# barbararoessle/e2e_multi_view_matching

Hardware: NVIDIA H100
Metric: view-tuples/sec @1024 kpts 5-view (higher is better)
Workload: dtype f32 via split operands on the tensor cores (fp16x3 / tf32x3, fp32-faithful) / f64 pose kernels

## Files before the change

e2e_multi_view_matching_b200/csrc/gemm_tc.cu:

```cuda
#include <cstring>
#include <map>
#include <mutex>
#include <tuple>
#include <cuda_fp16.h>
#include "common.cuh"
#include "kernels.cuh"
#include "tc_common.cuh"

namespace {

constexpr int BM = 128;
constexpr int PRODUCER_WARP = 8;
constexpr int NTHREADS = 384;
constexpr int PRODUCER_REGS = 40, CONSUMER_REGS = 232;
enum { W_RAW = 0, W_TF32 = 1, W_F16 = 2 };

template <int BN, int NPASS, int WM>
struct Cfg {
  static constexpr int BK = WM == W_F16 ? 64 : 32;
  static constexpr int A_BYTES = BM * BK * 4;
  static constexpr int W_PLANE = BN * 128;
  static constexpr int PLANES = NPASS == 3 ? 2 : 1;
  static constexpr int STAGE_BYTES = A_BYTES + PLANES * W_PLANE;
  static constexpr int TMA_BYTES = A_BYTES + (WM == W_RAW ? 1 : PLANES) * W_PLANE;
  static constexpr int STAGES = (196608 / STAGE_BYTES) < 6 ? (196608 / STAGE_BYTES) : 6;
  static constexpr bool STAGED = BN == 128 && NPASS == 3 && WM != W_RAW;
  static constexpr int OUT_BYTES = STAGED ? 2 * 16384 : 0;
  static constexpr int SMEM_BYTES = STAGES * STAGE_BYTES + OUT_BYTES + 1024  + 256 ;
  static_assert(SMEM_BYTES <= 232448, "over the sm_90 dynamic shared memory opt-in limit");
};

struct GArgs {
  const float* bias;
  const float* R; int ldr;
  float* C; int ldc;
  int M, N, K, K1;
  float alpha;
  int relu;
  float* VT; int vt_col0; int n_pad;
  float* KLO; float* VTLO;
  __half* KH16; __half* KL16; __half* VH16; __half* VL16;
  int tiles_m, tiles_n;
  int ksplit;
  int stage;
};

struct StoreMaps {
  CUtensorMap c, r, p[4];
};

struct ScoreTab {
  int n_pairs, batch, n_views, n_pad;
  int a[MVM_MAX_PAIRS], b[MVM_MAX_PAIRS], m[MVM_MAX_PAIRS], n[MVM_MAX_PAIRS];
  float* scores[MVM_MAX_PAIRS];
};

__device__ __forceinline__ float tf32_hi(float x) {
  return __uint_as_float((__float_as_uint(x) + 0x1000u) & 0xffffe000u);
}
__device__ __forceinline__ void split_pack_h(float x0, float x1, uint32_t& hi, uint32_t& lo) {
  const __half2 h = __floats2half2_rn(x0, x1);
  const float2 hf = __half22float2(h);
  const __half2 l = __floats2half2_rn(x0 - hf.x, x1 - hf.y);
  hi = *reinterpret_cast<const uint32_t*>(&h);
  lo = *reinterpret_cast<const uint32_t*>(&l);
}
__device__ __forceinline__ void sts_f2(uint32_t a, float2 v) {
  asm volatile("st.shared.v2.f32 [%0], {%1, %2};" ::"r"(a), "f"(v.x), "f"(v.y) : "memory");
}
__device__ __forceinline__ void sts_u32(uint32_t a, uint32_t v) {
  asm volatile("st.shared.b32 [%0], %1;" ::"r"(a), "r"(v) : "memory");
}
__device__ __forceinline__ float2 lds_f2(uint32_t a) {
  float2 v;
  asm volatile("ld.shared.v2.f32 {%0, %1}, [%2];" : "=f"(v.x), "=f"(v.y) : "r"(a) : "memory");
  return v;
}
__device__ __forceinline__ void fence_afrag(uint32_t (&a)[4][4]) {
#pragma unroll
  for (int i = 0; i < 4; ++i)
#pragma unroll
    for (int e = 0; e < 4; ++e) asm volatile("" : "+r"(a[i][e])::"memory");
}

template <int BN, int NPASS, int WM, bool SCORE>
__global__ void __launch_bounds__(NTHREADS, 1)
gemm_wg_kernel(const __grid_constant__ CUtensorMap tmA, const __grid_constant__ CUtensorMap tmA2,
               const __grid_constant__ CUtensorMap tmWhi, const __grid_constant__ CUtensorMap tmWlo,
               const __grid_constant__ GArgs g, const __grid_constant__ ScoreTab st,
               const __grid_constant__ StoreMaps sm) {
  using C_ = Cfg<BN, NPASS, WM>;
  static_assert(NPASS == 3 || WM == W_RAW, "single pass reads the raw W");
  constexpr int BK = C_::BK, STAGES = C_::STAGES, A_BYTES = C_::A_BYTES, W_PLANE = C_::W_PLANE;
  constexpr int STAGE_BYTES = C_::STAGE_BYTES;
  constexpr int KSTEPS = 4;
  constexpr bool PIPE = BN == 128;
  constexpr bool STAGED = C_::STAGED && !SCORE;
  extern __shared__ uint8_t smem_raw[];
  uint8_t* smem = reinterpret_cast<uint8_t*>((reinterpret_cast<uintptr_t>(smem_raw) + 1023) & ~uintptr_t(1023));
  uint8_t* obuf = smem + STAGES * STAGE_BYTES;
  uint64_t* full = reinterpret_cast<uint64_t*>(obuf + C_::OUT_BYTES);
  uint64_t* empty = full + STAGES;
  uint64_t* ostaged = empty + STAGES;
  uint64_t* ofree = ostaged + 2;

  const int warp = threadIdx.x >> 5, lane = threadIdx.x & 31;
  const int nk = SCORE ? g.K / BK : g.K / BK / g.ksplit;
  const int per_prob = g.tiles_m * g.tiles_n;
  const int n_tiles = SCORE ? per_prob * st.n_pairs * st.batch : per_prob * g.ksplit;
  auto decode = [&](int tile, int& m0, int& n0, int& a_row, int& w_row, int& prob) {
    prob = tile / per_prob;
    const int r = tile % per_prob;
    m0 = (r / g.tiles_n) * BM; n0 = (r % g.tiles_n) * BN;
    if (!SCORE) {
      a_row = m0; w_row = n0;
    } else {
      const int p = prob / st.batch, bi = prob % st.batch;
      a_row = (bi * st.n_views + st.a[p]) * st.n_pad + m0;
      w_row = (bi * st.n_views + st.b[p]) * st.n_pad + n0;
    }
  };
  auto tile_kind = [&](int n0) {
    if (g.VT && n0 >= g.vt_col0) return -1;
    if (g.KH16 && n0 >= 256) return 1;
    if (g.KLO && n0 >= 256 && n0 < 512) return 2;
    return 0;
  };

  if (threadIdx.x == 0) {
    for (int s = 0; s < STAGES; ++s) {
      tc::mbar_init(full + s, 1);
      tc::mbar_init(empty + s, 256);
    }
    if (STAGED)
      for (int b = 0; b < 2; ++b) {
        tc::mbar_init(ostaged + b, 256);
        tc::mbar_init(ofree + b, 1);
      }
    tc::fence_barrier_init();
  }
  __syncthreads();

  if (warp >= PRODUCER_WARP) {
    asm volatile("setmaxnreg.dec.sync.aligned.u32 %0;" ::"n"(PRODUCER_REGS));
    if (STAGED && g.stage && warp == PRODUCER_WARP + 1 && lane == 0) {
      tc::prefetch_tmap(&sm.c);
      if (g.R) tc::prefetch_tmap(&sm.r);
      if (g.KH16)
        for (int i = 0; i < 4; ++i) tc::prefetch_tmap(&sm.p[i]);
      if (g.KLO) tc::prefetch_tmap(&sm.p[0]);
      auto hand_back = [&](uint32_t u, int tile, int q) {
        uint64_t* bar = ofree + (u & 1);
        if (!g.R) {
          tc::mbar_arrive(bar);
        } else if (tile < n_tiles) {
          int m0, n0, a_row, w_row, prob;
          decode(tile, m0, n0, a_row, w_row, prob);
          tc::mbar_arrive_expect_tx(bar, 16384);
          tc::tma_load_2d(obuf + (u & 1) * 16384, &sm.r, bar, n0 + 32 * q, m0);
        }
      };
      hand_back(0, blockIdx.x, 0);
      hand_back(1, blockIdx.x, 1);
      uint32_t u = 0;
      for (int tile = blockIdx.x; tile < n_tiles; tile += gridDim.x) {
        int m0, n0, a_row, w_row, prob;
        decode(tile, m0, n0, a_row, w_row, prob);
        const int kind = tile_kind(n0);
        if (kind < 0) continue;
        const int rounds = kind == 2 ? 8 : 4;
        for (int j = 0; j < rounds; ++j, ++u) {
          const uint8_t* buf = obuf + (u & 1) * 16384;
          tc::mbar_wait(ostaged + (u & 1), (u >> 1) & 1);
          if (kind == 0) {
            tc::tma_store_2d(&sm.c, buf, n0 + 32 * j, m0 + prob * g.tiles_m * BM);
          } else if (kind == 1) {
            const bool v = n0 >= 512;
            tc::tma_store_2d(&sm.p[(v ? 2 : 0) + (j & 1)], buf, n0 - (v ? 512 : 256) + 64 * (j >> 1), m0);
          } else {
            if (j & 1) tc::tma_store_2d(&sm.p[0], buf, n0 - 256 + 32 * (j >> 1), m0);
            else tc::tma_store_2d(&sm.c, buf, n0 + 32 * (j >> 1), m0);
          }
          tc::tma_store_commit();
          tc::tma_store_wait_read<0>();
          hand_back(u + 2, j < 2 ? tile : tile + gridDim.x, (j + 2) & 3);
        }
      }
      tc::tma_store_wait_all();
    }
    if (warp == PRODUCER_WARP && lane == 0) {
      tc::prefetch_tmap(&tmA); tc::prefetch_tmap(&tmA2); tc::prefetch_tmap(&tmWhi); tc::prefetch_tmap(&tmWlo);
      uint32_t it = 0;
      for (int tile = blockIdx.x; tile < n_tiles; tile += gridDim.x) {
        int m0, n0, a_row, w_row, prob;
        decode(tile, m0, n0, a_row, w_row, prob);
        for (int kt = 0; kt < nk; ++kt, ++it) {
          const int s = it % STAGES;
          tc::mbar_wait(empty + s, ((it / STAGES) & 1) ^ 1);
          tc::mbar_arrive_expect_tx(full + s, C_::TMA_BYTES);
          uint8_t* sp = smem + s * STAGE_BYTES;
          const int k = kt * BK + (SCORE ? 0 : prob * nk * BK);
          if (k < g.K1) tc::tma_load_2d(sp, &tmA, full + s, k, a_row);
          else tc::tma_load_2d(sp, &tmA2, full + s, k - g.K1, a_row);
          if (WM == W_F16) {
            if (k < g.K1) tc::tma_load_2d(sp + 16384, &tmA, full + s, k + 32, a_row);
            else tc::tma_load_2d(sp + 16384, &tmA2, full + s, k + 32 - g.K1, a_row);
          }
          tc::tma_load_2d(sp + A_BYTES, &tmWhi, full + s, k, w_row);
          if (WM != W_RAW) tc::tma_load_2d(sp + A_BYTES + W_PLANE, &tmWlo, full + s, k, w_row);
        }
      }
    }
    return;
  }

  asm volatile("setmaxnreg.inc.sync.aligned.u32 %0;" ::"n"(CONSUMER_REGS));
  const int wg = warp >> 2, wq = warp & 3;
  const int gr = lane >> 2, tq = lane & 3;
  const int row0 = wg * 64 + wq * 16 + gr;
  float acc[BN / 2];
  uint32_t ahi0[KSTEPS][4], alo0[KSTEPS][4], ahi1[KSTEPS][4], alo1[KSTEPS][4];

  auto prep = [&](uint32_t it, uint32_t (&ahi)[KSTEPS][4], uint32_t (&alo)[KSTEPS][4]) {
      const int s = it % STAGES;
      tc::mbar_wait(full + s, (it / STAGES) & 1);
      uint8_t* sp = smem + s * STAGE_BYTES;
      if (WM == W_RAW && NPASS == 3) {
        float4* w = reinterpret_cast<float4*>(sp + A_BYTES);
        float4* wl = reinterpret_cast<float4*>(sp + A_BYTES + W_PLANE);
#pragma unroll 4
        for (int i = threadIdx.x; i < BN * 32 / 4; i += 256) {
          const float4 x = w[i];
          float4 h;
          h.x = tc::tf32_rn(x.x); h.y = tc::tf32_rn(x.y); h.z = tc::tf32_rn(x.z); h.w = tc::tf32_rn(x.w);
          w[i] = h;
          wl[i] = make_float4(tc::tf32_rn(x.x - h.x), tc::tf32_rn(x.y - h.y), tc::tf32_rn(x.z - h.z), tc::tf32_rn(x.w - h.w));
        }
        tc::fence_proxy_async();
        asm volatile("bar.sync 1, 256;" ::: "memory");
      }
      const uint8_t* ar = sp + row0 * 128;
#pragma unroll
      for (int kk = 0; kk < KSTEPS; ++kk) {
        if (WM == W_F16) {
          const uint8_t* ab = ar + (kk >> 1) * 16384;
          const int ch = 4 * (kk & 1) + (tq >> 1), wo = (tq & 1) * 8;
          const float2 x0 = *reinterpret_cast<const float2*>(ab + ((ch ^ gr) << 4) + wo);
          const float2 x1 = *reinterpret_cast<const float2*>(ab + 1024 + ((ch ^ gr) << 4) + wo);
          const float2 x2 = *reinterpret_cast<const float2*>(ab + (((ch + 2) ^ gr) << 4) + wo);
          const float2 x3 = *reinterpret_cast<const float2*>(ab + 1024 + (((ch + 2) ^ gr) << 4) + wo);
          split_pack_h(x0.x, x0.y, ahi[kk][0], alo[kk][0]);
          split_pack_h(x1.x, x1.y, ahi[kk][1], alo[kk][1]);
          split_pack_h(x2.x, x2.y, ahi[kk][2], alo[kk][2]);
          split_pack_h(x3.x, x3.y, ahi[kk][3], alo[kk][3]);
        } else {
          float x[4];
          x[0] = *reinterpret_cast<const float*>(ar + (((2 * kk) ^ gr) << 4) + tq * 4);
          x[1] = *reinterpret_cast<const float*>(ar + 1024 + (((2 * kk) ^ gr) << 4) + tq * 4);
          x[2] = *reinterpret_cast<const float*>(ar + (((2 * kk + 1) ^ gr) << 4) + tq * 4);
          x[3] = *reinterpret_cast<const float*>(ar + 1024 + (((2 * kk + 1) ^ gr) << 4) + tq * 4);
#pragma unroll
          for (int e = 0; e < 4; ++e) {
            if (NPASS == 3) {
              const float h = tf32_hi(x[e]);
              ahi[kk][e] = __float_as_uint(h);
              alo[kk][e] = __float_as_uint(tf32_hi(x[e] - h));
            } else {
              ahi[kk][e] = __float_as_uint(x[e]);
            }
          }
        }
      }
  };
  auto issue = [&](uint32_t it, const uint32_t (&ahi)[KSTEPS][4], const uint32_t (&alo)[KSTEPS][4]) {
      const uint32_t whi = tc::smem_u32(smem + (it % STAGES) * STAGE_BYTES + A_BYTES);
      tc::wgmma_fence();
#pragma unroll
      for (int kk = 0; kk < KSTEPS; ++kk) {
#pragma unroll
        for (int nh = 0; nh < BN / 128; ++nh) {
          float* d = acc + nh * 64;
          const uint32_t wb = whi + nh * 16384 + kk * 32;
          if (WM == W_F16) {
            tc::wgmma_f16_rs<128, 0>(d, ahi[kk], tc::make_sw128_desc(wb));
            tc::wgmma_f16_rs<128, 0>(d, ahi[kk], tc::make_sw128_desc(wb + W_PLANE));
            tc::wgmma_f16_rs<128, 0>(d, alo[kk], tc::make_sw128_desc(wb));
          } else {
            tc::wgmma_tf32_rs<128>(d, ahi[kk], tc::make_sw128_desc(wb));
            if (NPASS == 3) {
              tc::wgmma_tf32_rs<128>(d, ahi[kk], tc::make_sw128_desc(wb + W_PLANE));
              tc::wgmma_tf32_rs<128>(d, alo[kk], tc::make_sw128_desc(wb));
            }
          }
        }
      }
      tc::wgmma_commit();
  };
  auto keep = [&](uint32_t (&ahi)[KSTEPS][4], uint32_t (&alo)[KSTEPS][4]) {
    fence_afrag(ahi);
    if (NPASS == 3) fence_afrag(alo);
  };

  auto stage_round = [&](uint32_t u, int n0, int i0, int ni, int mode, int plane) {
    const uint32_t buf = tc::smem_u32(obuf + (u & 1) * 16384);
    float2 bv[8];
#pragma unroll
    for (int c = 0; c < ni; ++c) {
      const int n = n0 + 8 * (i0 + c) + 2 * tq;
      bv[c] = g.bias ? make_float2(__ldg(g.bias + n), __ldg(g.bias + n + 1)) : make_float2(0.f, 0.f);
    }
    tc::mbar_wait(ofree + (u & 1), (u >> 1) & 1);
#pragma unroll
    for (int c = 0; c < ni; ++c) {
      const int i = i0 + c;
#pragma unroll
      for (int hh = 0; hh < 2; ++hh) {
        const int r = row0 + 8 * hh;
        float x0 = __fmul_rn(g.alpha, acc[4 * i + 2 * hh]), x1 = __fmul_rn(g.alpha, acc[4 * i + 2 * hh + 1]);
        if (g.bias) { x0 = __fadd_rn(x0, bv[c].x); x1 = __fadd_rn(x1, bv[c].y); }
        if (g.relu) { x0 = fmaxf(x0, 0.f); x1 = fmaxf(x1, 0.f); }
        if (mode == 1) {
          uint32_t hi, lo;
          split_pack_h(x0, x1, hi, lo);
          sts_u32(buf + r * 128 + ((c ^ (r & 7)) << 4) + 4 * tq, plane ? lo : hi);
        } else {
          const uint32_t p = buf + r * 128 + (((2 * c + (tq >> 1)) ^ (r & 7)) << 4) + 8 * (tq & 1);
          if (mode == 2) {
            const float h0 = tf32_hi(x0), h1 = tf32_hi(x1);
            sts_f2(p, plane ? make_float2(tf32_hi(x0 - h0), tf32_hi(x1 - h1)) : make_float2(h0, h1));
          } else {
            if (g.R) { const float2 rv = lds_f2(p); x0 = __fadd_rn(x0, rv.x); x1 = __fadd_rn(x1, rv.y); }
            sts_f2(p, make_float2(x0, x1));
          }
        }
      }
    }
    tc::fence_proxy_async();
    tc::mbar_arrive(ostaged + (u & 1));
  };

  uint32_t it = 0, u = 0;
  for (int tile = blockIdx.x; tile < n_tiles; tile += gridDim.x) {
    int m0, n0, a_row, w_row, prob;
    decode(tile, m0, n0, a_row, w_row, prob);
#pragma unroll
    for (int i = 0; i < BN / 2; ++i) acc[i] = 0.f;
    if constexpr (PIPE) {
      prep(it, ahi0, alo0);
      for (int kt = 0; kt < nk; kt += 2) {
        issue(it + kt, ahi0, alo0);
        tc::wgmma_wait<1>();
        keep(ahi1, alo1);
        if (kt > 0) tc::mbar_arrive(empty + (it + kt - 1) % STAGES);
        if (kt + 1 < nk) {
          prep(it + kt + 1, ahi1, alo1);
          issue(it + kt + 1, ahi1, alo1);
          tc::wgmma_wait<1>();
          keep(ahi0, alo0);
          tc::mbar_arrive(empty + (it + kt) % STAGES);
          if (kt + 2 < nk) prep(it + kt + 2, ahi0, alo0);
        }
      }
      tc::wgmma_wait<0>();
      tc::fence_acc<BN>(acc);
      keep(ahi0, alo0);
      keep(ahi1, alo1);
      tc::mbar_arrive(empty + (it + nk - 1) % STAGES);
    } else {
      for (int kt = 0; kt < nk; ++kt) {
        prep(it + kt, ahi0, alo0);
        issue(it + kt, ahi0, alo0);
        tc::wgmma_wait<0>();
        tc::fence_acc<BN>(acc);
        keep(ahi0, alo0);
        tc::mbar_arrive(empty + (it + kt) % STAGES);
      }
    }
    it += nk;

    if (SCORE) {
      const int p = prob / st.batch, bi = prob % st.batch;
      const int pm = st.m[p], pn = st.n[p];
      float* Cp = st.scores[p] + (long long)bi * (pm + 1) * (pn + 1);
#pragma unroll
      for (int hh = 0; hh < 2; ++hh) {
        const int gm = m0 + row0 + 8 * hh;
        if (gm >= pm) continue;
#pragma unroll
        for (int i = 0; i < BN / 8; ++i) {
          const int gn = n0 + 8 * i + 2 * tq;
          if (gn < pn) Cp[(long long)gm * (pn + 1) + gn] = g.alpha * acc[4 * i + 2 * hh];
          if (gn + 1 < pn) Cp[(long long)gm * (pn + 1) + gn + 1] = g.alpha * acc[4 * i + 2 * hh + 1];
        }
      }
      continue;
    }
    if constexpr (STAGED) {
      const int kind = g.stage ? tile_kind(n0) : -1;
      if (kind >= 0) {
#pragma unroll
        for (int j = 0; j < 8; ++j) {
          if (kind == 1) {
            if (j < 4) stage_round(u + j, n0, 8 * (j >> 1), 8, 1, j & 1);
          } else if (kind == 2) {
            stage_round(u + j, n0, 4 * (j >> 1), 4, 2, j & 1);
          } else if (j < 4) {
            stage_round(u + j, n0, 4 * j, 4, 0, 0);
          }
        }
        u += kind == 2 ? 8 : 4;
        continue;
      }
    }
    auto put = [&](int m, int n, float x0, float x1) {
      if (g.VT && n >= g.vt_col0) {
        const int slab = m / g.n_pad, ii = m % g.n_pad;
        const long long off = ((long long)slab * (g.N - g.vt_col0) + (n - g.vt_col0)) * g.n_pad + ii;
        if (g.VTLO) {
          const float h0 = tf32_hi(x0), h1 = tf32_hi(x1);
          g.VT[off] = h0; g.VT[off + g.n_pad] = h1;
          g.VTLO[off] = tf32_hi(x0 - h0); g.VTLO[off + g.n_pad] = tf32_hi(x1 - h1);
        } else {
          g.VT[off] = x0; g.VT[off + g.n_pad] = x1;
        }
      } else if (g.KH16 && n >= 256) {
        const bool is_v = n >= 512;
        const long long o = (long long)m * 256 + n - (is_v ? 512 : 256);
        uint32_t hi, lo;
        split_pack_h(x0, x1, hi, lo);
        *reinterpret_cast<uint32_t*>((is_v ? g.VH16 : g.KH16) + o) = hi;
        *reinterpret_cast<uint32_t*>((is_v ? g.VL16 : g.KL16) + o) = lo;
      } else if (g.KLO && n >= 256 && n < 512) {
        const float h0 = tf32_hi(x0), h1 = tf32_hi(x1);
        *reinterpret_cast<float2*>(g.C + (long long)m * g.ldc + n) = make_float2(h0, h1);
        *reinterpret_cast<float2*>(g.KLO + (long long)m * 256 + n - 256) = make_float2(tf32_hi(x0 - h0), tf32_hi(x1 - h1));
      } else {
        const long long c_row = m + (long long)prob * g.tiles_m * BM;
        *reinterpret_cast<float2*>(g.C + c_row * g.ldc + n) = make_float2(x0, x1);
      }
    };
    if constexpr (PIPE) {
      constexpr int ICH = 8;
#pragma unroll
      for (int i0 = 0; i0 < BN / 8; i0 += ICH) {
        float2 bv[ICH], rv[ICH][2];
#pragma unroll
        for (int c = 0; c < ICH; ++c) {
          const int n = n0 + 8 * (i0 + c) + 2 * tq;
          bv[c] = g.bias ? make_float2(__ldg(g.bias + n), __ldg(g.bias + n + 1)) : make_float2(0.f, 0.f);
#pragma unroll
          for (int hh = 0; hh < 2; ++hh) {
            const int m = m0 + row0 + 8 * hh;
            rv[c][hh] = g.R && m < g.M ? __ldg(reinterpret_cast<const float2*>(g.R + (long long)m * g.ldr + n))
                                       : make_float2(0.f, 0.f);
          }
        }
#pragma unroll
        for (int c = 0; c < ICH; ++c) {
          const int i = i0 + c, n = n0 + 8 * i + 2 * tq;
#pragma unroll
          for (int hh = 0; hh < 2; ++hh) {
            const int m = m0 + row0 + 8 * hh;
            if (m >= g.M) continue;
            float x0 = g.alpha * acc[4 * i + 2 * hh], x1 = g.alpha * acc[4 * i + 2 * hh + 1];
            if (g.bias) { x0 += bv[c].x; x1 += bv[c].y; }
            if (g.relu) { x0 = fmaxf(x0, 0.f); x1 = fmaxf(x1, 0.f); }
            if (g.R) { x0 += rv[c][hh].x; x1 += rv[c][hh].y; }
            put(m, n, x0, x1);
          }
        }
      }
    } else {
#pragma unroll
      for (int hh = 0; hh < 2; ++hh) {
        const int m = m0 + row0 + 8 * hh;
        if (m >= g.M) continue;
#pragma unroll
        for (int i = 0; i < BN / 8; ++i) {
          const int n = n0 + 8 * i + 2 * tq;
          float x0 = g.alpha * acc[4 * i + 2 * hh], x1 = g.alpha * acc[4 * i + 2 * hh + 1];
          if (g.bias) { x0 += __ldg(g.bias + n); x1 += __ldg(g.bias + n + 1); }
          if (g.relu) { x0 = fmaxf(x0, 0.f); x1 = fmaxf(x1, 0.f); }
          if (g.R) {
            const float2 r = __ldg(reinterpret_cast<const float2*>(g.R + (long long)m * g.ldr + n));
            x0 += r.x; x1 += r.y;
          }
          put(m, n, x0, x1);
        }
      }
    }
  }
}

template <int BN, int NPASS, int WM, bool SCORE>
int launch_wg(const CUtensorMap* tA, const CUtensorMap* tA2, const CUtensorMap* tWhi, const CUtensorMap* tWlo,
              const GArgs& g, const ScoreTab& st, long long n_tiles, bool persistent, cudaStream_t stream,
              const StoreMaps& sm) {
  using C_ = Cfg<BN, NPASS, WM>;
  if (!tA || !tA2 || !tWhi || !tWlo) return MVM_ERR_LAUNCH;
  if (n_tiles <= 0) return MVM_OK;
  if (cudaFuncSetAttribute(gemm_wg_kernel<BN, NPASS, WM, SCORE>, cudaFuncAttributeMaxDynamicSharedMemorySize,
                           C_::SMEM_BYTES) != cudaSuccess)
    return MVM_ERR_LAUNCH;
  const int n_sm = mvm_dev_info().n_sm;
  const int grid = (persistent && n_tiles > n_sm) ? n_sm : (int)n_tiles;
  gemm_wg_kernel<BN, NPASS, WM, SCORE><<<grid, NTHREADS, C_::SMEM_BYTES, stream>>>(*tA, *tA2, *tWhi, *tWlo, g, st, sm);
  MVM_CHECK_LAUNCH();
  return MVM_OK;
}

StoreMaps no_store_maps() {
  StoreMaps none;
  memset(&none, 0, sizeof(none));
  return none;
}

GArgs make_args(const GemmDesc& d, float* VT, int vt_col0, int n_pad, float* KLO, float* VTLO, int bn) {
  GArgs g;
  memset(&g, 0, sizeof(g));
  g.bias = d.bias; g.R = d.R; g.ldr = d.ldr; g.C = d.C; g.ldc = d.ldc; g.M = d.M; g.N = d.N; g.K = d.K;
  g.K1 = d.K1; g.alpha = d.alpha; g.relu = d.relu; g.VT = VT; g.vt_col0 = vt_col0; g.n_pad = n_pad;
  g.KLO = KLO; g.VTLO = VTLO;
  g.tiles_m = mvm_div_up(d.M, BM); g.tiles_n = d.N / bn; g.ksplit = 1;
  return g;
}

ScoreTab no_scores() {
  ScoreTab none;
  memset(&none, 0, sizeof(none));
  return none;
}

template <int BN, int NPASS, int WM>
int launch_cfg(const GemmDesc& d, float* VT, int vt_col0, int n_pad, float* KLO, float* VTLO, bool persistent,
               cudaStream_t stream) {
  const CUtensorMap* tA = mvm_get_tmap_2d(d.A, d.M, d.K1, d.lda, BM);
  const CUtensorMap* tA2 = d.A2 ? mvm_get_tmap_2d(d.A2, d.M, d.K - d.K1, d.lda2, BM) : tA;
  const CUtensorMap* tW = mvm_get_tmap_2d(WM == W_TF32 ? d.Whi : d.W, d.N, d.K, d.ldw, BN);
  const CUtensorMap* tWlo = WM == W_TF32 ? mvm_get_tmap_2d(d.Wlo, d.N, d.K, d.ldw, BN) : tW;
  const GArgs g = make_args(d, VT, vt_col0, n_pad, KLO, VTLO, BN);
  return launch_wg<BN, NPASS, WM, false>(tA, tA2, tW, tWlo, g, no_scores(), (long long)g.tiles_m * g.tiles_n, persistent,
                                         stream, no_store_maps());
}


__global__ void split_planes_kernel(const float4* __restrict__ x, float4* __restrict__ hi, float4* __restrict__ lo,
                                    long long n4) {
  for (long long i = blockIdx.x * (long long)blockDim.x + threadIdx.x; i < n4; i += (long long)gridDim.x * blockDim.x) {
    const float4 v = x[i];
    float4 h, l;
    h.x = tf32_hi(v.x); h.y = tf32_hi(v.y); h.z = tf32_hi(v.z); h.w = tf32_hi(v.w);
    l.x = tf32_hi(v.x - h.x); l.y = tf32_hi(v.y - h.y); l.z = tf32_hi(v.z - h.z); l.w = tf32_hi(v.w - h.w);
    hi[i] = h;
    lo[i] = l;
  }
}

__global__ void splitk_reduce_kernel(const float4* __restrict__ slabs, float* __restrict__ C, int M, int N4, int ldc, int S) {
  const long long i = blockIdx.x * (long long)blockDim.x + threadIdx.x;
  if (i >= (long long)M * N4) return;
  const int m = (int)(i / N4), n4 = (int)(i % N4);
  float4 a = slabs[i];
  for (int s = 1; s < S; ++s) {
    const float4 b = slabs[(long long)s * M * N4 + i];
    a.x += b.x; a.y += b.y; a.z += b.z; a.w += b.w;
  }
  *reinterpret_cast<float4*>(C + (long long)m * ldc + 4 * n4) = a;
}

typedef CUresult (*EncodeFn)(CUtensorMap*, CUtensorMapDataType, cuuint32_t, void*, const cuuint64_t*,
                             const cuuint64_t*, const cuuint32_t*, const cuuint32_t*, CUtensorMapInterleave,
                             CUtensorMapSwizzle, CUtensorMapL2promotion, CUtensorMapFloatOOBfill);
EncodeFn get_encode() {
  static EncodeFn fn = nullptr;
  if (!fn) {
    void* p = nullptr;
    cudaDriverEntryPointQueryResult qres;
    if (cudaGetDriverEntryPoint("cuTensorMapEncodeTiled", &p, cudaEnableDefault, &qres) != cudaSuccess || !p) return nullptr;
    fn = reinterpret_cast<EncodeFn>(p);
  }
  return fn;
}
typedef std::tuple<const void*, long long, long long, long long, long long, long long, int> TmKey;
std::map<TmKey, CUtensorMap*> g_tmaps;
std::mutex g_tmap_mu;

}

const CUtensorMap* mvm_get_tmap_3d(const float* base, long long slabs, long long rows, long long cols,
                                   long long ld_row, long long ld_slab, int box_rows) {
  std::lock_guard<std::mutex> lk(g_tmap_mu);
  TmKey key(base, slabs, rows, cols, ld_row, ld_slab, box_rows);
  auto it = g_tmaps.find(key);
  if (it != g_tmaps.end()) return it->second;
  EncodeFn enc = get_encode();
  if (!enc) return nullptr;
  CUtensorMap* tm = new CUtensorMap;
  const int rank = slabs > 0 ? 3 : 2;
  cuuint64_t dims[3] = {(cuuint64_t)cols, (cuuint64_t)rows, (cuuint64_t)(slabs > 0 ? slabs : 1)};
  cuuint64_t strides[2] = {(cuuint64_t)ld_row * 4, (cuuint64_t)ld_slab * 4};
  cuuint32_t box[3] = {32, (cuuint32_t)box_rows, 1};
  cuuint32_t estr[3] = {1, 1, 1};
  CUresult r = enc(tm, CU_TENSOR_MAP_DATA_TYPE_FLOAT32, rank, const_cast<float*>(base), dims, strides, box, estr,
                   CU_TENSOR_MAP_INTERLEAVE_NONE, CU_TENSOR_MAP_SWIZZLE_128B, CU_TENSOR_MAP_L2_PROMOTION_L2_128B,
                   CU_TENSOR_MAP_FLOAT_OOB_FILL_NONE);
  if (r != CUDA_SUCCESS) {
    fprintf(stderr, "[mvm_b200] cuTensorMapEncodeTiled failed (%d) rows=%lld cols=%lld ld=%lld\n", (int)r, rows, cols, ld_row);
    delete tm;
    return nullptr;
  }
  g_tmaps[key] = tm;
  return tm;
}

const CUtensorMap* mvm_get_tmap_2d(const float* base, long long rows, long long cols, long long ld, int box_rows) {
  return mvm_get_tmap_3d(base, 0, rows, cols, ld, 0, box_rows);
}

const CUtensorMap* mvm_get_tmap_2d_f16(const void* base, long long rows, long long cols, long long ld, int box_rows) {
  std::lock_guard<std::mutex> lk(g_tmap_mu);
  TmKey key(base, -16, rows, cols, ld, 0, box_rows);
  auto it = g_tmaps.find(key);
  if (it != g_tmaps.end()) return it->second;
  EncodeFn enc = get_encode();
  if (!enc) return nullptr;
  CUtensorMap* tm = new CUtensorMap;
  cuuint64_t dims[2] = {(cuuint64_t)cols, (cuuint64_t)rows};
  cuuint64_t strides[1] = {(cuuint64_t)ld * 2};
  cuuint32_t box[2] = {64, (cuuint32_t)box_rows};
  cuuint32_t estr[2] = {1, 1};
  CUresult r = enc(tm, CU_TENSOR_MAP_DATA_TYPE_FLOAT16, 2, const_cast<void*>(base), dims, strides, box, estr,
                   CU_TENSOR_MAP_INTERLEAVE_NONE, CU_TENSOR_MAP_SWIZZLE_128B, CU_TENSOR_MAP_L2_PROMOTION_L2_128B,
                   CU_TENSOR_MAP_FLOAT_OOB_FILL_NONE);
  if (r != CUDA_SUCCESS) {
    fprintf(stderr, "[mvm_b200] cuTensorMapEncodeTiled (f16) failed (%d) rows=%lld cols=%lld ld=%lld\n", (int)r, rows, cols, ld);
    delete tm;
    return nullptr;
  }
  g_tmaps[key] = tm;
  return tm;
}


int g_gemm_bn = 256;
extern "C" void mvm_debug_set_gemm_tile(int bn) { g_gemm_bn = bn == 256 ? 256 : 128; }
int g_gemm_persist = 1;
extern "C" void mvm_debug_set_gemm_kernel(int persistent) { g_gemm_persist = persistent ? 1 : 0; }

int mvm_default_gemm_tile() { return g_gemm_bn; }
int mvm_default_gemm_persistent() { return g_gemm_persist; }

int launch_gemm_tc(const GemmDesc& d, int n_pass, float* VT, int vt_col0, int n_pad, cudaStream_t stream,
                   float* KLO, float* VTLO, int gemm_tile, int gemm_persist) {
  if (gemm_tile < 0) gemm_tile = g_gemm_bn;
  if (gemm_persist < 0) gemm_persist = g_gemm_persist;
  MVM_REQUIRE(gemm_desc_valid(d, GEMM_TC_TF32));
  MVM_REQUIRE(d.W || (n_pass == 3 && d.Whi && d.Wlo));
  MVM_REQUIRE(mvm_aligned(KLO, 8));
  MvmProfScope prof__(MVM_TAG_GEMM, stream);
  if (gemm_persist && n_pass == 3 && d.Whi && d.Wlo) return launch_gemm_tc_persist(d, VT, vt_col0, n_pad, KLO, VTLO, stream);
  if (gemm_tile == 256 && d.N % 256 == 0) {
    if (n_pass == 3 && d.Whi && d.Wlo) return launch_cfg<256, 3, W_TF32>(d, VT, vt_col0, n_pad, KLO, VTLO, false, stream);
    if (n_pass == 1) return launch_cfg<256, 1, W_RAW>(d, VT, vt_col0, n_pad, nullptr, nullptr, false, stream);
  }
  if (n_pass == 3 && d.Whi && d.Wlo) return launch_cfg<128, 3, W_TF32>(d, VT, vt_col0, n_pad, KLO, VTLO, false, stream);
  if (n_pass == 3) return launch_cfg<128, 3, W_RAW>(d, VT, vt_col0, n_pad, KLO, VTLO, false, stream);
  return launch_cfg<128, 1, W_RAW>(d, VT, vt_col0, n_pad, nullptr, nullptr, false, stream);
}

int launch_gemm_tc_persist(const GemmDesc& d, float* VT, int vt_col0, int n_pad, float* KLO, float* VTLO,
                           cudaStream_t stream, const HalfPlanes* hp, int ksplit, float* slabs) {
  MVM_REQUIRE(ksplit >= 1 && (ksplit == 1 || (slabs && d.M % BM == 0 && d.K % (32 * ksplit) == 0 && !d.Whi16 && !d.bias && !d.R && !d.A2 &&
                                               !d.relu && !VT && !KLO && !hp)));
  const bool f16 = d.Whi16 != nullptr && d.Wlo16 != nullptr && d.K % 64 == 0 && d.K1 % 64 == 0 && d.wscale > 0.f;
  MVM_REQUIRE(f16 ? gemm_desc_valid(d, GEMM_TC_F16) : gemm_desc_valid(d, GEMM_TC_TF32) && d.Whi && d.Wlo);
  MVM_REQUIRE(mvm_aligned(KLO, 8) && mvm_aligned(slabs, 16));
  MVM_REQUIRE(!hp || (mvm_aligned(hp->kh, 4) && mvm_aligned(hp->kl, 4) && mvm_aligned(hp->vh, 4) && mvm_aligned(hp->vl, 4)));
  const CUtensorMap* tA = mvm_get_tmap_2d(d.A, d.M, d.K1, d.lda, BM);
  const CUtensorMap* tA2 = d.A2 ? mvm_get_tmap_2d(d.A2, d.M, d.K - d.K1, d.lda2, BM) : tA;
  GArgs g = make_args(d, VT, vt_col0, n_pad, KLO, VTLO, 128);
  if (ksplit > 1) { g.C = slabs; g.ldc = d.N; }
  g.ksplit = ksplit;
  if (hp) {
    g.KH16 = (__half*)hp->kh; g.KL16 = (__half*)hp->kl; g.VH16 = (__half*)hp->vh; g.VL16 = (__half*)hp->vl;
  }
  const long long n_tiles = (long long)g.tiles_m * g.tiles_n * ksplit;
  StoreMaps sm = no_store_maps();
  const void* planes[4] = {g.KH16, g.KL16, g.VH16, g.VL16};
  bool stage = mvm_aligned(g.C, 16) && mvm_aligned(g.R, 16) && mvm_aligned(g.KLO, 16) && (!g.VT || g.vt_col0 % 128 == 0) &&
               (!g.R || (!g.KH16 && !g.KLO && !g.VT));
  for (const void* p : planes) stage = stage && mvm_aligned(p, 16);
  if (stage) {
    const CUtensorMap* c = mvm_get_tmap_2d(g.C, (long long)(ksplit - 1) * g.tiles_m * BM + g.M, g.N, g.ldc, BM);
    const CUtensorMap* r = g.R ? mvm_get_tmap_2d(g.R, g.M, g.N, g.ldr, BM) : c;
    if (!c || !r) return MVM_ERR_LAUNCH;
    sm.c = *c; sm.r = *r;
    for (int i = 0; i < 4; ++i) {
      const CUtensorMap* p = g.KH16 ? mvm_get_tmap_2d_f16(planes[i], g.M, 256, 256, BM)
                                    : g.KLO && i == 0 ? mvm_get_tmap_2d(g.KLO, g.M, 256, 256, BM) : c;
      if (!p) return MVM_ERR_LAUNCH;
      sm.p[i] = *p;
    }
    g.stage = 1;
  }
  if (f16) {
    g.alpha = d.alpha / d.wscale;
    const CUtensorMap* tWhi = mvm_get_tmap_2d_f16(d.Whi16, d.N, d.K, d.ldw, 128);
    const CUtensorMap* tWlo = mvm_get_tmap_2d_f16(d.Wlo16, d.N, d.K, d.ldw, 128);
    return launch_wg<128, 3, W_F16, false>(tA, tA2, tWhi, tWlo, g, no_scores(), n_tiles, true, stream, sm);
  }
  const CUtensorMap* tWhi = mvm_get_tmap_2d(d.Whi, d.N, d.K, d.ldw, 128);
  const CUtensorMap* tWlo = mvm_get_tmap_2d(d.Wlo, d.N, d.K, d.ldw, 128);
  return launch_wg<128, 3, W_TF32, false>(tA, tA2, tWhi, tWlo, g, no_scores(), n_tiles, true, stream, sm);
}

int launch_splitk_reduce(const float* slabs, float* C, int M, int N, int ldc, int ksplit, cudaStream_t stream) {
  MVM_REQUIRE(N % 4 == 0 && ldc % 4 == 0 && mvm_aligned(slabs, 16) && mvm_aligned(C, 16));
  const long long n = (long long)M * (N / 4);
  splitk_reduce_kernel<<<(unsigned)((n + 255) / 256), 256, 0, stream>>>(reinterpret_cast<const float4*>(slabs), C, M, N / 4, ldc, ksplit);
  MVM_CHECK_LAUNCH();
  return MVM_OK;
}

int launch_score_gemm_tc(const float* mdesc, float* hi, float* lo, int n_pad, const PairTable& tab, int batch,
                         float alpha, cudaStream_t stream) {
  MvmProfScope prof__(MVM_TAG_SCORE, stream);
  const int n_sm = mvm_dev_info().n_sm;
  const long long rows = (long long)batch * tab.n_views * n_pad;
  split_planes_kernel<<<n_sm * 4, 256, 0, stream>>>(reinterpret_cast<const float4*>(mdesc), reinterpret_cast<float4*>(hi),
                                                    reinterpret_cast<float4*>(lo), rows * 256 / 4);
  MVM_CHECK_LAUNCH();
  const CUtensorMap* tA = mvm_get_tmap_2d(mdesc, rows, 256, 256, BM);
  const CUtensorMap* tWhi = mvm_get_tmap_2d(hi, rows, 256, 256, 128);
  const CUtensorMap* tWlo = mvm_get_tmap_2d(lo, rows, 256, 256, 128);
  ScoreTab st = no_scores();
  st.n_pairs = tab.n_pairs; st.batch = batch; st.n_views = tab.n_views; st.n_pad = n_pad;
  int max_m = 0, max_n = 0;
  for (int p = 0; p < tab.n_pairs; ++p) {
    st.a[p] = tab.a[p]; st.b[p] = tab.b[p]; st.m[p] = tab.m[p]; st.n[p] = tab.n[p]; st.scores[p] = tab.scores[p];
    max_m = tab.m[p] > max_m ? tab.m[p] : max_m;
    max_n = tab.n[p] > max_n ? tab.n[p] : max_n;
  }
  GArgs g;
  memset(&g, 0, sizeof(g));
  g.K = 256; g.K1 = 256; g.alpha = alpha; g.ksplit = 1;
  g.tiles_m = mvm_div_up(max_m, BM); g.tiles_n = mvm_div_up(max_n, 128);
  const long long n_tiles = (long long)g.tiles_m * g.tiles_n * tab.n_pairs * batch;
  return launch_wg<128, 3, W_TF32, true>(tA, tA, tWhi, tWlo, g, st, n_tiles, true, stream, no_store_maps());
}
```

Measured before the change: 213.9.

## Ping-pong consumer warpgroups across tiles to overlap epilogue with MMA

For the staged BN=128 three-pass GEMM, each consumer warpgroup now owns whole 128-row tiles on alternating iterations, with doubled accumulators (two 64-row halves). Named barriers order the main loops and the epilogues of the two warpgroups, so one warpgroup's epilogue can run while the other issues wgmma. This is meant to hide epilogue and store latency behind tensor core work. It doubles the accumulator register footprint per thread, which could cause spills, and the barrier handshakes are intricate.

Result: faster. 216.8 (median of 6 runs) (+1.4%).

```diff
diff --git a/e2e_multi_view_matching_b200/csrc/gemm_tc.cu b/e2e_multi_view_matching_b200/csrc/gemm_tc.cu
--- a/e2e_multi_view_matching_b200/csrc/gemm_tc.cu
+++ b/e2e_multi_view_matching_b200/csrc/gemm_tc.cu
@@ -76,11 +76,19 @@
   asm volatile("ld.shared.v2.f32 {%0, %1}, [%2];" : "=f"(v.x), "=f"(v.y) : "r"(a) : "memory");
   return v;
 }
-__device__ __forceinline__ void fence_afrag(uint32_t (&a)[4][4]) {
-#pragma unroll
-  for (int i = 0; i < 4; ++i)
+template <int R>
+__device__ __forceinline__ void fence_afrag(uint32_t (&a)[R][4]) {
+#pragma unroll
+  for (int i = 0; i < R; ++i)
 #pragma unroll
     for (int e = 0; e < 4; ++e) asm volatile("" : "+r"(a[i][e])::"memory");
+}
+constexpr int MAIN_BAR = 2, EPI_BAR = 4;
+__device__ __forceinline__ void named_bar_sync(int id, int n) {
+  asm volatile("bar.sync %0, %1;" ::"r"(id), "r"(n) : "memory");
+}
+__device__ __forceinline__ void named_bar_arrive(int id, int n) {
+  asm volatile("bar.arrive %0, %1;" ::"r"(id), "r"(n) : "memory");
 }
 
 template <int BN, int NPASS, int WM, bool SCORE>
@@ -96,6 +104,9 @@
   constexpr int KSTEPS = 4;
   constexpr bool PIPE = BN == 128;
   constexpr bool STAGED = C_::STAGED && !SCORE;
+  constexpr bool PING = STAGED;
+  constexpr int NH = PING ? 2 : 1;
+  constexpr int CONSUMERS = PING ? 128 : 256;
   extern __shared__ uint8_t smem_raw[];
   uint8_t* smem = reinterpret_cast<uint8_t*>((reinterpret_cast<uintptr_t>(smem_raw) + 1023) & ~uintptr_t(1023));
   uint8_t* obuf = smem + STAGES * STAGE_BYTES;
@@ -130,11 +141,11 @@
   if (threadIdx.x == 0) {
     for (int s = 0; s < STAGES; ++s) {
       tc::mbar_init(full + s, 1);
-      tc::mbar_init(empty + s, 256);
+      tc::mbar_init(empty + s, CONSUMERS);
     }
     if (STAGED)
       for (int b = 0; b < 2; ++b) {
-        tc::mbar_init(ostaged + b, 256);
+        tc::mbar_init(ostaged + b, CONSUMERS);
         tc::mbar_init(ofree + b, 1);
       }
     tc::fence_barrier_init();
@@ -217,10 +228,40 @@
   asm volatile("setmaxnreg.inc.sync.aligned.u32 %0;" ::"n"(CONSUMER_REGS));
   const int wg = warp >> 2, wq = warp & 3;
   const int gr = lane >> 2, tq = lane & 3;
-  const int row0 = wg * 64 + wq * 16 + gr;
-  float acc[BN / 2];
+  const int row0 = (PING ? 0 : wg * 64) + wq * 16 + gr;
+  float acc[BN / 2 * NH];
   uint32_t ahi0[KSTEPS][4], alo0[KSTEPS][4], ahi1[KSTEPS][4], alo1[KSTEPS][4];
 
+  auto split_kstep = [&](const uint8_t* ar, int kk, uint32_t (&ahi)[4], uint32_t (&alo)[4]) {
+    if (WM == W_F16) {
+      const uint8_t* ab = ar + (kk >> 1) * 16384;
+      const int ch = 4 * (kk & 1) + (tq >> 1), wo = (tq & 1) * 8;
+      const float2 x0 = *reinterpret_cast<const float2*>(ab + ((ch ^ gr) << 4) + wo);
+      const float2 x1 = *reinterpret_cast<const float2*>(ab + 1024 + ((ch ^ gr) << 4) + wo);
+      const float2 x2 = *reinterpret_cast<const float2*>(ab + (((ch + 2) ^ gr) << 4) + wo);
+      const float2 x3 = *reinterpret_cast<const float2*>(ab + 1024 + (((ch + 2) ^ gr) << 4) + wo);
+      split_pack_h(x0.x, x0.y, ahi[0], alo[0]);
+      split_pack_h(x1.x, x1.y, ahi[1], alo[1]);
+      split_pack_h(x2.x, x2.y, ahi[2], alo[2]);
+      split_pack_h(x3.x, x3.y, ahi[3], alo[3]);
+    } else {
+      float x[4];
+      x[0] = *reinterpret_cast<const float*>(ar + (((2 * kk) ^ gr) << 4) + tq * 4);
+      x[1] = *reinterpret_cast<const float*>(ar + 1024 + (((2 * kk) ^ gr) << 4) + tq * 4);
+      x[2] = *reinterpret_cast<const float*>(ar + (((2 * kk + 1) ^ gr) << 4) + tq * 4);
+      x[3] = *reinterpret_cast<const float*>(ar + 1024 + (((2 * kk + 1) ^ gr) << 4) + tq * 4);
+#pragma unroll
+      for (int e = 0; e < 4; ++e) {
+        if (NPASS == 3) {
+          const float h = tf32_hi(x[e]);
+          ahi[e] = __float_as_uint(h);
+          alo[e] = __float_as_uint(tf32_hi(x[e] - h));
+        } else {
+          ahi[e] = __float_as_uint(x[e]);
+        }
+      }
+    }
+  };
   auto prep = [&](uint32_t it, uint32_t (&ahi)[KSTEPS][4], uint32_t (&alo)[KSTEPS][4]) {
       const int s = it % STAGES;
       tc::mbar_wait(full + s, (it / STAGES) & 1);
@@ -239,38 +280,8 @@
         tc::fence_proxy_async();
         asm volatile("bar.sync 1, 256;" ::: "memory");
       }
-      const uint8_t* ar = sp + row0 * 128;
-#pragma unroll
-      for (int kk = 0; kk < KSTEPS; ++kk) {
-        if (WM == W_F16) {
-          const uint8_t* ab = ar + (kk >> 1) * 16384;
-          const int ch = 4 * (kk & 1) + (tq >> 1), wo = (tq & 1) * 8;
-          const float2 x0 = *reinterpret_cast<const float2*>(ab + ((ch ^ gr) << 4) + wo);
-          const float2 x1 = *reinterpret_cast<const float2*>(ab + 1024 + ((ch ^ gr) << 4) + wo);
-          const float2 x2 = *reinterpret_cast<const float2*>(ab + (((ch + 2) ^ gr) << 4) + wo);
-          const float2 x3 = *reinterpret_cast<const float2*>(ab + 1024 + (((ch + 2) ^ gr) << 4) + wo);
-          split_pack_h(x0.x, x0.y, ahi[kk][0], alo[kk][0]);
-          split_pack_h(x1.x, x1.y, ahi[kk][1], alo[kk][1]);
-          split_pack_h(x2.x, x2.y, ahi[kk][2], alo[kk][2]);
-          split_pack_h(x3.x, x3.y, ahi[kk][3], alo[kk][3]);
-        } else {
-          float x[4];
-          x[0] = *reinterpret_cast<const float*>(ar + (((2 * kk) ^ gr) << 4) + tq * 4);
-          x[1] = *reinterpret_cast<const float*>(ar + 1024 + (((2 * kk) ^ gr) << 4) + tq * 4);
-          x[2] = *reinterpret_cast<const float*>(ar + (((2 * kk + 1) ^ gr) << 4) + tq * 4);
-          x[3] = *reinterpret_cast<const float*>(ar + 1024 + (((2 * kk + 1) ^ gr) << 4) + tq * 4);
-#pragma unroll
-          for (int e = 0; e < 4; ++e) {
-            if (NPASS == 3) {
-              const float h = tf32_hi(x[e]);
-              ahi[kk][e] = __float_as_uint(h);
-              alo[kk][e] = __float_as_uint(tf32_hi(x[e] - h));
-            } else {
-              ahi[kk][e] = __float_as_uint(x[e]);
-            }
-          }
-        }
-      }
+#pragma unroll
+      for (int kk = 0; kk < KSTEPS; ++kk) split_kstep(sp + row0 * 128, kk, ahi[kk], alo[kk]);
   };
   auto issue = [&](uint32_t it, const uint32_t (&ahi)[KSTEPS][4], const uint32_t (&alo)[KSTEPS][4]) {
       const uint32_t whi = tc::smem_u32(smem + (it % STAGES) * STAGE_BYTES + A_BYTES);
@@ -314,9 +325,9 @@
     for (int c = 0; c < ni; ++c) {
       const int i = i0 + c;
 #pragma unroll
-      for (int hh = 0; hh < 2; ++hh) {
-        const int r = row0 + 8 * hh;
-        float x0 = __fmul_rn(g.alpha, acc[4 * i + 2 * hh]), x1 = __fmul_rn(g.alpha, acc[4 * i + 2 * hh + 1]);
+      for (int hh = 0; hh < 2 * NH; ++hh) {
+        const int r = row0 + 64 * (hh >> 1) + 8 * (hh & 1), a = 64 * (hh >> 1) + 4 * i + 2 * (hh & 1);
+        float x0 = __fmul_rn(g.alpha, acc[a]), x1 = __fmul_rn(g.alpha, acc[a + 1]);
         if (g.bias) { x0 = __fadd_rn(x0, bv[c].x); x1 = __fadd_rn(x1, bv[c].y); }
         if (g.relu) { x0 = fmaxf(x0, 0.f); x1 = fmaxf(x1, 0.f); }
         if (mode == 1) {
@@ -339,13 +350,85 @@
     tc::mbar_arrive(ostaged + (u & 1));
   };
 
+  auto tile_rounds = [&](int n0) {
+    const int kind = g.stage ? tile_kind(n0) : -1;
+    return kind < 0 ? 0 : kind == 2 ? 8 : 4;
+  };
+  if (PING && wg == 1) {
+    named_bar_arrive(MAIN_BAR + 0, 256);
+    named_bar_arrive(EPI_BAR + 0, 256);
+  }
+
   uint32_t it = 0, u = 0;
-  for (int tile = blockIdx.x; tile < n_tiles; tile += gridDim.x) {
+  for (int tile = blockIdx.x, ti = 0; tile < n_tiles; tile += gridDim.x, ++ti) {
     int m0, n0, a_row, w_row, prob;
     decode(tile, m0, n0, a_row, w_row, prob);
-#pragma unroll
-    for (int i = 0; i < BN / 2; ++i) acc[i] = 0.f;
-    if constexpr (PIPE) {
+    const bool last = tile + gridDim.x >= n_tiles;
+    if (PING && (ti & 1) != wg) {
+      it += nk;
+      u += tile_rounds(n0);
+      continue;
+    }
+#pragma unroll
+    for (int i = 0; i < BN / 2 * NH; ++i) acc[i] = 0.f;
+    if constexpr (PING) {
+      uint32_t fhi0[NH][4], flo0[NH][4], fhi1[NH][4], flo1[NH][4];
+      auto split_step = [&](uint32_t itk, int kk, uint32_t (&fhi)[NH][4], uint32_t (&flo)[NH][4]) {
+        const uint8_t* ar = smem + (itk % STAGES) * STAGE_BYTES + row0 * 128;
+#pragma unroll
+        for (int h = 0; h < NH; ++h) split_kstep(ar + h * 64 * 128, kk, fhi[h], flo[h]);
+      };
+      auto issue_step = [&](uint32_t itk, int kk, const uint32_t (&fhi)[NH][4], const uint32_t (&flo)[NH][4]) {
+        const uint32_t wb = tc::smem_u32(smem + (itk % STAGES) * STAGE_BYTES + A_BYTES) + kk * 32;
+        tc::wgmma_fence();
+#pragma unroll
+        for (int pass = 0; pass < 3; ++pass)
+#pragma unroll
+          for (int h = 0; h < NH; ++h) {
+            const uint32_t* a = pass < 2 ? fhi[h] : flo[h];
+            const uint64_t desc = tc::make_sw128_desc(pass == 1 ? wb + W_PLANE : wb);
+            if (WM == W_F16) tc::wgmma_f16_rs<128, 0>(acc + 64 * h, a, desc);
+            else tc::wgmma_tf32_rs<128>(acc + 64 * h, a, desc);
+          }
+        tc::wgmma_commit();
+      };
+      auto keep_step = [&](uint32_t (&fhi)[NH][4], uint32_t (&flo)[NH][4]) {
+        fence_afrag(fhi);
+        fence_afrag(flo);
+      };
+      named_bar_sync(MAIN_BAR + wg, 256);
+      tc::mbar_wait(full + it % STAGES, (it / STAGES) & 1);
+      split_step(it, 0, fhi0, flo0);
+      for (int kt = 0; kt < nk; ++kt) {
+        const uint32_t itk = it + kt;
+        issue_step(itk, 0, fhi0, flo0);
+        tc::wgmma_wait<1>();
+        keep_step(fhi1, flo1);
+        if (kt > 0) tc::mbar_arrive(empty + (itk - 1) % STAGES);
+        split_step(itk, 1, fhi1, flo1);
+        issue_step(itk, 1, fhi1, flo1);
+        tc::wgmma_wait<1>();
+        keep_step(fhi0, flo0);
+        split_step(itk, 2, fhi0, flo0);
+        issue_step(itk, 2, fhi0, flo0);
+        tc::wgmma_wait<1>();
+        keep_step(fhi1, flo1);
+        split_step(itk, 3, fhi1, flo1);
+        issue_step(itk, 3, fhi1, flo1);
+        if (kt + 1 == nk && !last) named_bar_arrive(MAIN_BAR + (wg ^ 1), 256);
+        tc::wgmma_wait<1>();
+        keep_step(fhi0, flo0);
+        if (kt + 1 < nk) {
+          tc::mbar_wait(full + (itk + 1) % STAGES, ((itk + 1) / STAGES) & 1);
+          split_step(itk + 1, 0, fhi0, flo0);
+        }
+      }
+      tc::wgmma_wait<0>();
+      tc::fence_acc<2 * BN>(acc);
+      keep_step(fhi0, flo0);
+      keep_step(fhi1, flo1);
+      tc::mbar_arrive(empty + (it + nk - 1) % STAGES);
+    } else if constexpr (PIPE) {
       prep(it, ahi0, alo0);
       for (int kt = 0; kt < nk; kt += 2) {
         issue(it + kt, ahi0, alo0);
@@ -395,6 +478,10 @@
       }
       continue;
     }
+    if constexpr (PING) named_bar_sync(EPI_BAR + wg, 256);
+    auto epilogue_done = [&] {
+      if (PING && !last) named_bar_arrive(EPI_BAR + (wg ^ 1), 256);
+    };
     if constexpr (STAGED) {
       const int kind = g.stage ? tile_kind(n0) : -1;
       if (kind >= 0) {
@@ -409,6 +496,7 @@
           }
         }
         u += kind == 2 ? 8 : 4;
+        epilogue_done();
         continue;
       }
     }
@@ -442,6 +530,8 @@
     if constexpr (PIPE) {
       constexpr int ICH = 8;
 #pragma unroll
+      for (int h = 0; h < NH; ++h)
+#pragma unroll
       for (int i0 = 0; i0 < BN / 8; i0 += ICH) {
         float2 bv[ICH], rv[ICH][2];
 #pragma unroll
@@ -450,7 +540,7 @@
           bv[c] = g.bias ? make_float2(__ldg(g.bias + n), __ldg(g.bias + n + 1)) : make_float2(0.f, 0.f);
 #pragma unroll
           for (int hh = 0; hh < 2; ++hh) {
-            const int m = m0 + row0 + 8 * hh;
+            const int m = m0 + row0 + 64 * h + 8 * hh;
             rv[c][hh] = g.R && m < g.M ? __ldg(reinterpret_cast<const float2*>(g.R + (long long)m * g.ldr + n))
                                        : make_float2(0.f, 0.f);
           }
@@ -460,9 +550,9 @@
           const int i = i0 + c, n = n0 + 8 * i + 2 * tq;
 #pragma unroll
           for (int hh = 0; hh < 2; ++hh) {
-            const int m = m0 + row0 + 8 * hh;
+            const int m = m0 + row0 + 64 * h + 8 * hh;
             if (m >= g.M) continue;
-            float x0 = g.alpha * acc[4 * i + 2 * hh], x1 = g.alpha * acc[4 * i + 2 * hh + 1];
+            float x0 = g.alpha * acc[64 * h + 4 * i + 2 * hh], x1 = g.alpha * acc[64 * h + 4 * i + 2 * hh + 1];
             if (g.bias) { x0 += bv[c].x; x1 += bv[c].y; }
             if (g.relu) { x0 = fmaxf(x0, 0.f); x1 = fmaxf(x1, 0.f); }
             if (g.R) { x0 += rv[c][hh].x; x1 += rv[c][hh].y; }
@@ -489,6 +579,7 @@
         }
       }
     }
+    epilogue_done();
   }
 }
 
```
